# mdolab/dafoam

Hardware: NVIDIA H100
Metric: dRdWTPsi_GCells_per_s (higher is better)
Workload: dtype f64

## Files before the change

dafoam_b200/csrc/acc.hpp:

```cpp
#pragma once
#include "views.hpp"

namespace dab
{

struct GAcc
{
    MeshView m;
    StateView s;
    RecordView r;
    AdjView a;
    PsiView x;
    double *yU, *yP, *yN, *yPhi;

    DAB_HD int maxCF() const { return m.maxCF; }
    DAB_HD int nIF() const { return m.nIF; }
    DAB_HD FaceRef face(int c, int k) const { return faceOf(m, c, k); }
    template <int NF>
    DAB_HD void faceRow(int c, int* e, int* n) const
    {
        _Pragma("unroll") for (int k = 0; k < NF; k++)
        {
            e[k] = m.cellFaces[(size_t)k * m.nC + c];
            n[k] = m.cellNbr[(size_t)k * m.nC + c];
        }
    }
    DAB_HD bool ghost(int n) const { return n >= m.nC; }
    DAB_HD int patch(int f) const { return m.bPatch[f - m.nIF]; }
    DAB_HD void Sf(int f, double* v) const { v[0] = m.Sx[f]; v[1] = m.Sy[f]; v[2] = m.Sz[f]; }
    DAB_HD void kv(int f, double* v) const { v[0] = m.kx[f]; v[1] = m.ky[f]; v[2] = m.kz[f]; }
    DAB_HD void Cf(int f, double* v) const { v[0] = m.Cfx[f]; v[1] = m.Cfy[f]; v[2] = m.Cfz[f]; }
    DAB_HD double magSf(int f) const { return m.magSf[f]; }
    DAB_HD double w(int f) const { return m.w[f]; }
    DAB_HD double delta(int f) const { return m.delta[f]; }
    DAB_HD double phi(int f) const { return s.phi[f]; }
    DAB_HD double xphi(int f) const { return x.phi[f]; }
    DAB_HD double V(int c) const { return m.V[c]; }
    DAB_HD double yWall(int c) const { return m.yWall[c]; }
    DAB_HD double C(int c, int j) const { return (j == 0 ? m.Cx : (j == 1 ? m.Cy : m.Cz))[c]; }
    DAB_HD double U(int c, int j) const { return s.U[3 * c + j]; }
    DAB_HD double p(int c) const { return s.p[c]; }
    DAB_HD double nt(int c) const { return s.nt[c]; }
    DAB_HD double xU(int c, int j) const { return x.U[3 * c + j]; }
    DAB_HD double xp(int c) const { return x.p[c]; }
    DAB_HD double xnt(int c) const { return x.nt[c]; }
    DAB_HD double nut(int c) const { return r.nut[c]; }
    DAB_HD double gU(int c, int i) const { return r.gU[(size_t)i * m.nCtot + c]; }
    DAB_HD double gP(int c, int i) const { return r.gP[(size_t)i * m.nCtot + c]; }
    DAB_HD double gNt(int c, int i) const { return r.gNt[(size_t)i * m.nCtot + c]; }
    DAB_HD double rAU(int c) const { return r.rAU[c]; }
    DAB_HD double HbyA(int c, int j) const { return r.HbyA[(size_t)j * m.nCtot + c]; }
    DAB_HD double D0(int c) const { return r.D0[c]; }
    DAB_HD double flag(int c) const { return r.flag[c]; }
    DAB_HD double mt(int c, int j) const { return a.mt[(size_t)j * m.nCtot + c]; }
    DAB_HD double Dn(int c) const { return a.Dn[c]; }
    DAB_HD double Udir(int c, int j) const { return a.Udir[(size_t)j * m.nC + c]; }
    DAB_HD double pdir(int c) const { return a.pdir[c]; }
    DAB_HD double gPb(int c, int i) const { return a.gPb[(size_t)i * m.nCtot + c]; }
    DAB_HD double gUb(int c, int i) const { return a.gUb[(size_t)i * m.nCtot + c]; }
    DAB_HD double gNtb(int c, int i) const { return a.gNtb[(size_t)i * m.nCtot + c]; }
    DAB_HD double nutb(int c) const { return a.nutb[c]; }
    DAB_HD double U2(int c, int j) const { return a.U2[(size_t)j * m.nC + c]; }
    DAB_HD double nt2(int c) const { return a.nt2[c]; }
    DAB_HD void setMt(int c, int j, double v) const { a.mt[(size_t)j * m.nCtot + c] = v; }
    DAB_HD void setDn(int c, double v) const { a.Dn[c] = v; }
    DAB_HD void setUdir(int c, int j, double v) const { a.Udir[(size_t)j * m.nC + c] = v; }
    DAB_HD void setPdir(int c, double v) const { a.pdir[c] = v; }
    DAB_HD void setGPb(int c, int i, double v) const { a.gPb[(size_t)i * m.nCtot + c] = v; }
    DAB_HD void setGUb(int c, int i, double v) const { a.gUb[(size_t)i * m.nCtot + c] = v; }
    DAB_HD void setGNtb(int c, int i, double v) const { a.gNtb[(size_t)i * m.nCtot + c] = v; }
    DAB_HD void setNutb(int c, double v) const { a.nutb[c] = v; }
    DAB_HD void setU2(int c, int j, double v) const { a.U2[(size_t)j * m.nC + c] = v; }
// ... 14 lines not shown
```

dafoam_b200/csrc/rev_kernels.hpp:

```cpp
#pragma once
#include "views.hpp"
#include "acc.hpp"
#include "fwd_kernels.hpp"
#include <cmath>

namespace dab
{

DAB_HD double sgn(double x) { return x < 0.0 ? -1.0 : 1.0; }

DAB_HD void saSourceAdj(double nt, double nu, double y, const double* gU, const double* gN, double z, double& ntb, double* gUb, double* gNb, int fv3,
                        double* nub = nullptr)
{
    const double inu = frcp(nu);
    const double chi = nt * inu;
    const double c3 = chi * chi * chi, den1 = c3 + SA::Cv1c, iden1 = frcp(den1);
    const double fv1 = c3 * iden1;
    const double den = 1.0 + chi * fv1, iden = frcp(den);
    const double fv2 = 1.0 - chi * iden;
    const double w01 = 0.5 * (gU[3] - gU[1]), w02 = 0.5 * (gU[6] - gU[2]), w12 = 0.5 * (gU[7] - gU[5]);
    const double Q = w01 * w01 + w02 * w02 + w12 * w12;
    const double sQ = sqrt(Q);
    const double Omega = 2.0 * sQ;
    const double ky2 = (SA::kappa * y) * (SA::kappa * y), iky2 = frcp(ky2), iy2 = iky2 * (SA::kappa * SA::kappa);
// ... 228 lines not shown
    D0 = D1 + mt[0] * U[0] + mt[1] * U[1] + mt[2] * U[2];
}

template <int NF, int FEAT, class Acc>
DAB_HD void revBCell(const Acc& A, const Params& q, int c, bool gradOnly)
{
    const int schU = q.divU, schN = q.divNut;
    const double Uc[3] = {A.U(c, 0), A.U(c, 1), A.U(c, 2)};
    const double nuEc = A.nut(c) + q.nu;
    double gUc[9];
    for (int i = 0; i < 9; i++) gUc[i] = A.gU(c, i);
    const double ntc = q.turb ? A.nt(c) : 0.0;
    const double rsig = 1.0 / SA::sigma, rAl = frcp(q.alphaU);
    const double mtc[3] = {A.mt(c, 0), A.mt(c, 1), A.mt(c, 2)};
    const double Dnc = A.Dn(c), flc = A.flag(c);
    const double qc = (q.turb ? A.xnt(c) : 0.0) * (q.nrNut ? frcp(A.V(c)) : 1.0);

    double U2[3] = {0, 0, 0}, nt2 = 0.0, nuEb = 0.0, gUb[9], gNb[3] = {0, 0, 0};
    double refb[3] = {0, 0, 0};
    for (int i = 0; i < 9; i++) gUb[i] = 0.0;

    DAB_ACC_FACES(NF)
    int kb = NF > 0 ? NF : A.maxCF();
    _Pragma("unroll") for (int k = 0; k < (NF > 0 ? NF : A.maxCF()); k++)
    {
        const FaceRef fr = DAB_ACC_FACE(NF, k);
        if (fr.f < 0 || fr.bnd)
        {
            kb = k;
            break;
        }
        const int f = fr.f, n = fr.n;
        const double phi = A.phi(f), xphif = A.xphi(f);
        double Sv[3], kv[3], Cfv[3];
        A.Sf(f, Sv);
        A.kv(f, kv);
        A.Cf(f, Cfv);
        const double mS = A.magSf(f), dl = A.delta(f), wf = A.w(f);
        const double Un[3] = {A.U(n, 0), A.U(n, 1), A.U(n, 2)};
        const double nutn = A.nut(n), Dnn = A.Dn(n), fln = A.flag(n), Vn = A.V(n);
        const double mtn[3] = {A.mt(n, 0), A.mt(n, 1), A.mt(n, 2)};
        const double Cn[3] = {A.C(n, 0), A.C(n, 1), A.C(n, 2)};
        double gUn[9], gNn[3];
        for (int i = 0; i < 9; i++) gUn[i] = A.gU(n, i);
        const double ntn = q.turb ? A.nt(n) : 0.0, xntn = q.turb ? A.xnt(n) : 0.0;
        for (int i = 0; i < 3; i++) gNn[i] = q.turb ? A.gNt(n, i) : 0.0;
        const double Cc[3] = {A.C(c, 0), A.C(c, 1), A.C(c, 2)};
        double gNc[3];
        for (int i = 0; i < 3; i++) gNc[i] = q.turb ? A.gNt(c, i) : 0.0;
        const double mf = fr.s * phi;
        const double rmS = frcp(mS);
        double phib_acc = 0.0;
        const double wc = fr.s > 0 ? wf : 1.0 - wf, wn = 1.0 - wc;
        const bool pos0 = phi >= 0.0;
        const double wupc = fr.s > 0 ? (pos0 ? 1.0 : 0.0) : (pos0 ? 0.0 : 1.0);
        const double nuEn = nutn + q.nu;
        double D1c, soc, D0c, D1n, son, D0n;
        diagAdj(Dnc, flc, rAl, mtc, Uc, D1c, soc, D0c);
        diagAdj(Dnn, fln, rAl, mtn, Un, D1n, son, D0n);
        const bool ownUp = phi > 0.0;
        const bool cUp = fr.s > 0 ? ownUp : !ownUp;
        const double dC[3] = {Cfv[0] - Cc[0], Cfv[1] - Cc[1], Cfv[2] - Cc[2]};
        {
            const double wpc = schU == DIV_LINEAR ? wc : wupc;
            const double wpn = schU == DIV_LINEAR ? wn : 1.0 - wupc;
            const double gf = (wc * nuEc + wn * nuEn) * mS;
            const double g = gf * dl;
            const double offc = mf - wpc * mf - g;
            const double offn = -mf + wpn * mf - g;
            const double offbc = mtc[0] * Un[0] + mtc[1] * Un[1] + mtc[2] * Un[2] + sgn(offc) * soc;
            const double offbn = mtn[0] * Uc[0] + mtn[1] * Uc[1] + mtn[2] * Uc[2] + sgn(offn) * son;
            for (int j = 0; j < 3; j++) U2[j] += offn * mtn[j];
            const double abc = D0c - offbc, abn = D0n - offbn;
            double gb = abc + abn;
            double gfb = 0.0;
            const double lam[3] = {fr.s * (mtc[0] - mtn[0]), fr.s * (mtc[1] - mtn[1]), fr.s * (mtc[2] - mtn[2])};
            if (fr.s > 0)
            {
                const double mbc = -D0c + offbc + wpc * abc;
                const double mbn = -D0n + offbn + wpn * abn;
                phib_acc += mbc - mbn;
            }
            if (!(FEAT & 1))
            {
                if (schU == DIV_LINEAR_UPWIND)
                {
                    if (cUp)
                        for (int j = 0; j < 3; j++)
                            for (int i = 0; i < 3; i++) gUb[j * 3 + i] += dC[i] * phi * lam[j];
                    if (fr.s > 0)
                    {
                        double d[3];
                        for (int i = 0; i < 3; i++) d[i] = cUp ? dC[i] : Cfv[i] - Cn[i];
                        for (int j = 0; j < 3; j++)
                        {
                            const double gu0 = cUp ? gUc[j * 3 + 0] : gUn[j * 3 + 0], gu1 = cUp ? gUc[j * 3 + 1] : gUn[j * 3 + 1],
                                         gu2 = cUp ? gUc[j * 3 + 2] : gUn[j * 3 + 2];
                            phib_acc += (d[0] * gu0 + d[1] * gu1 + d[2] * gu2) * lam[j];
                        }
                    }
                }
            }
            else if (schU == DIV_LINEAR_UPWIND || schU == DIV_LINEAR_UPWIND_V)
            {
                double gu[9];
                for (int i = 0; i < 9; i++) gu[i] = cUp ? gUc[i] : gUn[i];
                double d[3];
                for (int i = 0; i < 3; i++) d[i] = cUp ? dC[i] : Cfv[i] - Cn[i];
                double corr[3], corrL[3], outb[3], corrb[3] = {0, 0, 0};
                for (int j = 0; j < 3; j++)
                {
                    corr[j] = d[0] * gu[j * 3 + 0] + d[1] * gu[j * 3 + 1] + d[2] * gu[j * 3 + 2];
                    outb[j] = phi * lam[j];
                }
                if ((FEAT & 1) && schU == DIV_LINEAR_UPWIND_V)
                {
                    const double cf = ownUp ? (1.0 - wf) : -wf;
                    double maxCorr[3], maxCorrb[3] = {0, 0, 0};
                    for (int j = 0; j < 3; j++) maxCorr[j] = cf * fr.s * (Un[j] - Uc[j]);
                    luvLimit(corr, maxCorr, corrL);
                    luvLimitAdj(corr, maxCorr, outb, corrb, maxCorrb);
                    for (int j = 0; j < 3; j++) U2[j] -= cf * fr.s * maxCorrb[j];
                }
                else
                    for (int j = 0; j < 3; j++) { corrL[j] = corr[j]; corrb[j] = outb[j]; }
                if (cUp)
                    for (int j = 0; j < 3; j++)
                        for (int i = 0; i < 3; i++) gUb[j * 3 + i] += dC[i] * corrb[j];
                if (fr.s > 0)
                    for (int j = 0; j < 3; j++) phib_acc += corrL[j] * lam[j];
            }
            for (int j = 0; j < 3; j++)
            {
                double cg = 0.0;
                for (int i = 0; i < 3; i++) cg += kv[i] * (wc * gUc[j * 3 + i] + wn * gUn[j * 3 + i]);
                gfb -= cg * lam[j];
                const double cgb = -gf * lam[j];
                for (int i = 0; i < 3; i++) gUb[j * 3 + i] += wc * kv[i] * cgb;
            }
            const double trc = gUc[0] + gUc[4] + gUc[8];
            double trb = 0.0;
            for (int j = 0; j < 3; j++)
            {
                const double tcb = -wc * lam[j];
                const double tcj = Sv[0] * gUc[0 * 3 + j] + Sv[1] * gUc[1 * 3 + j] + Sv[2] * gUc[2 * 3 + j] - (2.0 / 3.0) * trc * Sv[j];
                nuEb += tcb * tcj;
                for (int i = 0; i < 3; i++) gUb[i * 3 + j] += nuEc * Sv[i] * tcb;
                trb -= (2.0 / 3.0) * nuEc * Sv[j] * tcb;
            }
            gUb[0] += trb; gUb[4] += trb; gUb[8] += trb;
            nuEb += wc * mS * (dl * gb + gfb);
        }
        if (q.turb)
        {
            const double qn = xntn * (q.nrNut ? frcp(Vn) : 1.0);
            const double wpc = schN == DIV_LINEAR ? wc : wupc;
            const double wpn = schN == DIV_LINEAR ? wn : 1.0 - wupc;
            const double Gc = (ntc + q.nu) * rsig;
            const double gf = (wc * Gc + wn * (ntn + q.nu) * rsig) * mS;
            const double g = gf * dl;
            nt2 += qc * (wpc * mf + g - mf) + qn * (-mf + wpn * mf - g);
            const double gb = (qc - qn) * (ntc - ntn);
            double gfb = 0.0;
            const double lam = fr.s * (qc - qn);
            if (fr.s > 0) phib_acc += qc * (1.0 - wpc) * (ntn - ntc) - qn * (1.0 - wpn) * (ntc - ntn);
            if (schN == DIV_LINEAR_UPWIND)
            {
                if (cUp)
                    for (int i = 0; i < 3; i++) gNb[i] += dC[i] * phi * lam;
                if (fr.s > 0)
                {
                    double corr = 0.0;
                    for (int i = 0; i < 3; i++) corr += (cUp ? dC[i] * gNc[i] : (Cfv[i] - Cn[i]) * gNn[i]);
                    phib_acc += corr * lam;
                }
            }
            double cg = 0.0;
            for (int i = 0; i < 3; i++) cg += kv[i] * (wc * gNc[i] + wn * gNn[i]);
            gfb -= cg * lam;
            const double cgb = -gf * lam;
            for (int i = 0; i < 3; i++) gNb[i] += wc * kv[i] * cgb;
            nt2 += wc * mS * (dl * gb + gfb) * rsig;
        }
        if (!gradOnly)
        {
            if (fr.s > 0)
                A.setYPhi(f, (phib_acc - (q.nrPhi ? rmS : 1.0) * xphif) * phiRowScale(q, mS));
            else if (A.ghost(n))
                A.setYPhi(f, 0.0);
        }
    }
    _Pragma("unroll") for (int k = 0; k < (NF > 0 ? NF : A.maxCF()); k++)
    {
        if (k < kb) continue;
        const FaceRef fr = DAB_ACC_FACE(NF, k);
        if (fr.f < 0) break;
        const int f = fr.f;
        const double phi = A.phi(f), xphif = A.xphi(f);
        double Sv[3];
        A.Sf(f, Sv);
        const double mS = A.magSf(f), dl = A.delta(f);
        const int pa = A.patch(f);
        const double nutc = A.nut(c);
        const double mf = phi;
        const double rmS = frcp(mS);
        double D1c, soc, D0c;
// ... 390 lines not shown
```

dafoam_b200/csrc/solver.hpp:

```cpp
#pragma once
#include "backend.hpp"
#include "mesh.hpp"
#include "views.hpp"
#include "fwd_kernels.hpp"
#include "rev_kernels.hpp"
#include "tile_kernels.hpp"
#include "comp_kernels.hpp"
#include "comp_rev_kernels.hpp"
#include "krylov.hpp"
#include "primal_kernels.hpp"
#include "geom_kernels.hpp"
#include "comp_primal_kernels.hpp"
#include "launch_traits.hpp"
#include "partition.hpp"
#include "comm.hpp"
#include <chrono>
#include <cstdlib>
#include <cstdio>
#include <fstream>
#include <map>
#include <sys/stat.h>
#include <set>

namespace dab
// ... 135 lines not shown
    int pcExtraColourRadius = 0;
    int globalPCIters = 0;
    double richardsonOmega = 1.0;
    double gmresRelTol = 1e-6, gmresAbsTol = 1e-14, gmresTolDiff = 1e2, fdStep = 1e-6;
    std::string pcType = "ilu";
    std::string pcStorage = "fp64";
    int coarseAggregates = 0;
    int pcConLevel = 2;
    std::vector<FunctionDef> functions;
    std::vector<PatchVelocityDef> patchVelocities;
    std::vector<PatchVarDef> patchVars;
    FvSourceSpec fvSpec{};
    std::vector<std::string> diskNames;
    struct FvSourceParDef { std::string name, disk; std::vector<int> indices; };
    std::vector<FvSourceParDef> fvSourcePars;
    DevBuf<double> dFvS;
    struct MrfZone
    {
        bool on = false;
        std::string zone;
        double omega[3] = {0, 0, 0}, origin[3] = {0, 0, 0};
        std::vector<unsigned char> cell, type, faceIn;
    } mrf;
    DevBuf<unsigned char> dMrfCell, dMrfType, dMrfFaceIn;
    DevBuf<double> dMrfFlux;
    void updateMrfFlux()
    {
        if (mrf.on) be.launch(hm.nF, MrfFluxK{mv, dMrfFaceIn.p, dMrfFlux.p});
    }

    DevBuf<int32_t> dOwn, dNei, dCellFaces, dCellNbr, dBPatch;
    DevBuf<double> dS[3], dMagSf, dW, dDelta, dK[3], dCf[3], dV, dY;
    DevBuf<double> dC;
    MeshView mv;
    DevBuf<double> dWext, dU, dP, dNt, dPhi, dT;
    DevBuf<double> rRho, rNuL, rMuE, rAE, rHe, rEk, rGHe;
    DevBuf<double> aGHeb, aTdir, aCRho, aCNu, aCMuE, aCAE, aCHe, aCEk;
    StateView sv;
    DevBuf<double> rNut, rGU, rGP, rGNt, rRAU, rHbyA, rD0, rFlag;
    RecordView rv;
    DevBuf<double> aMt, aDn, aUdir, aPdir, aGPb, aGUb, aGNtb, aNutb, aU2, aNt2;
    AdjView av;
    DevBuf<double> dR, dX, dY2;
    bool recorded = false;
    Krylov kry;
    Comm comm;
    Halo halo;
    Partition part;
    DevBuf<double> psiP, psiN, psiPhi, psiT;

    TileMap tiles;
    DevBuf<int32_t> dTileCum, dTileGid, dTileTf, dTileTn;
    TileView tvw{};
    bool tilesOn = false;
    int tileCellsHint = 0;

    DevBuf<int32_t> dPfRanges;
    int pfChunks = 0;
    bool pfOn = false;

    bool fvSourceDirty = false;
    bool hex6 = false;
    int nCellStates() const { return 4 + (par.comp ? 1 : 0) + (par.turb ? 1 : 0); }
    int nDof() const { return nCellStates() * hm.nC + hm.nF; }
    void requireIncompressible(const char* what) const
    {
// ... 713 lines not shown
        (void)first;
        recorded = false;
    }

    void upload()
    {
        dOwn.upload(be, hm.own);
        dNei.upload(be, hm.nei);
        dCellFaces.upload(be, hm.cellFaces);
        hex6 = hm.maxCF == 6 && !(getenv("DAB_NOHEX6") && atoi(getenv("DAB_NOHEX6")) > 0);
        for (size_t i = 0; i < hm.cellFaces.size() && hex6; i++)
            if (hm.cellFaces[i] < 0) hex6 = false;
        hm.buildCellNbr();
        dCellNbr.upload(be, hm.cellNbr);
        dBPatch.upload(be, hm.bPatch);
        for (int k = 0; k < 3; k++)
        {
            dS[k].upload(be, hm.Sf[k]);
            dK[k].upload(be, hm.corr[k]);
            dCf[k].upload(be, hm.Cf[k]);
        }
        dC.alloc(be, (size_t)3 * hm.nCtot, false);
        for (int k = 0; k < 3; k++) be.h2d(dC.p + (size_t)k * hm.nCtot, hm.C[k].data(), (size_t)hm.nCtot * sizeof(double));
        dMagSf.upload(be, hm.magSf);
        dW.upload(be, hm.w);
        dDelta.upload(be, hm.delta);
        dV.upload(be, hm.V);
        dY.upload(be, hm.yWall);
        mv.nC = hm.nC; mv.nCtot = hm.nCtot; mv.nF = hm.nF; mv.nIF = hm.nIF; mv.nBF = hm.nBF; mv.maxCF = hm.maxCF;
        mv.own = dOwn.p; mv.nei = dNei.p; mv.cellFaces = dCellFaces.p; mv.cellNbr = dCellNbr.p; mv.bPatch = dBPatch.p;
        mv.Sx = dS[0].p; mv.Sy = dS[1].p; mv.Sz = dS[2].p; mv.magSf = dMagSf.p; mv.w = dW.p; mv.delta = dDelta.p;
        mv.kx = dK[0].p; mv.ky = dK[1].p; mv.kz = dK[2].p; mv.Cfx = dCf[0].p; mv.Cfy = dCf[1].p; mv.Cfz = dCf[2].p;
        mv.Cx = dC.p; mv.Cy = dC.p + hm.nCtot; mv.Cz = dC.p + 2 * (size_t)hm.nCtot; mv.V = dV.p; mv.yWall = dY.p;
        mv.fvS = nullptr;
        mv.mrfCell = nullptr; mv.mrfType = nullptr; mv.mrfFlux = nullptr;
        if (mrf.on)
        {
            dMrfCell.upload(be, mrf.cell);
            dMrfType.upload(be, mrf.type);
            dMrfFaceIn.upload(be, mrf.faceIn);
            dMrfFlux.alloc(be, hm.nF);
            for (int k = 0; k < 3; k++)
            {
                mv.mrfOmega[k] = mrf.omega[k];
                mv.mrfOrigin[k] = mrf.origin[k];
            }
            mv.mrfCell = dMrfCell.p; mv.mrfType = dMrfType.p; mv.mrfFlux = dMrfFlux.p;
            updateMrfFlux();
        }
        fvSourceDirty = fvSpec.nDisk > 0;
        const size_t nT = hm.nCtot, nC = hm.nC, nF = hm.nF, nd = nDof();
        dWext.alloc(be, nd);
        dU.alloc(be, 3 * nT); dP.alloc(be, nT); dNt.alloc(be, nT); dPhi.alloc(be, nF);
        sv.U = dU.p; sv.p = dP.p; sv.nt = dNt.p; sv.phi = dPhi.p; sv.T = nullptr;
        rv.rho = rv.nuL = rv.muE = rv.aE = rv.he = rv.Ek = rv.gHe = nullptr;
        if (par.comp)
        {
            dT.alloc(be, nT);
            sv.T = dT.p;
            rRho.alloc(be, nT); rNuL.alloc(be, nT); rMuE.alloc(be, nT); rAE.alloc(be, nT); rHe.alloc(be, nT); rEk.alloc(be, nT);
            rGHe.alloc(be, 3 * nT);
            rv.rho = rRho.p; rv.nuL = rNuL.p; rv.muE = rMuE.p; rv.aE = rAE.p; rv.he = rHe.p; rv.Ek = rEk.p; rv.gHe = rGHe.p;
        }
        rNut.alloc(be, nT); rGU.alloc(be, 9 * nT); rGP.alloc(be, 3 * nT); rGNt.alloc(be, 3 * nT);
        rRAU.alloc(be, nT); rHbyA.alloc(be, 3 * nT); rD0.alloc(be, nT); rFlag.alloc(be, nT);
        rv.nut = rNut.p; rv.gU = rGU.p; rv.gP = rGP.p; rv.gNt = rGNt.p; rv.rAU = rRAU.p; rv.HbyA = rHbyA.p; rv.D0 = rD0.p; rv.flag = rFlag.p;
// ... 107 lines not shown
        PfPlan pl;
        if (!pfOn) return pl;
        pl.nC = hm.nC;
        pl.nChunks = pfChunks;
        pl.ranges = dPfRanges.p;
        static const int ahead = getenv("DAB_PF_AHEAD") ? atoi(getenv("DAB_PF_AHEAD")) : 0;
        pl.ahead = ahead;
        const size_t nC = hm.nC;
        for (int k = 0; k < hm.maxCF && k < 6; k++)
        {
            pl.cell(mv.cellFaces + (size_t)k * nC, 4);
            pl.cell(mv.cellNbr + (size_t)k * nC, 4);
        }
        return pl;
    }
    PfPlan pfRevA(const PsiView& pv) const
    {
        PfPlan pl = pfBase();
        if (!pfOn) return pl;
        const size_t nT = hm.nCtot;
        pl.cell(sv.U, 24); pl.cell(pv.U, 24); pl.cell(pv.p, 8); pl.cell(mv.V, 8); pl.cell(sv.p, 8); pl.cell(rv.rAU, 8); pl.cell(rv.D0, 8);
        for (int j = 0; j < 3; j++) { pl.cell(rv.gP + j * nT, 8); pl.cell(rv.HbyA + j * nT, 8); }
        pl.face(mv.magSf, 8); pl.face(mv.delta, 8); pl.face(mv.Sx, 8); pl.face(mv.Sy, 8); pl.face(mv.Sz, 8); pl.face(pv.phi, 8);
        pl.face(mv.w, 8); pl.face(mv.kx, 8); pl.face(mv.ky, 8); pl.face(mv.kz, 8); pl.face(sv.phi, 8);
        return pl;
    }
    PfPlan pfRevB(const PsiView& pv) const
    {
        PfPlan pl = pfBase();
        if (!pfOn) return pl;
        const size_t nT = hm.nCtot;
        pl.cell(sv.U, 24); pl.cell(rv.nut, 8); pl.cell(mv.V, 8); pl.cell(av.Dn, 8); pl.cell(rv.flag, 8);
        for (int i = 0; i < 9; i++) pl.cell(rv.gU + i * nT, 8);
        for (int j = 0; j < 3; j++) { pl.cell(av.mt + j * nT, 8); pl.cell((j == 0 ? mv.Cx : (j == 1 ? mv.Cy : mv.Cz)), 8); }
        if (par.turb)
        {
            pl.cell(sv.nt, 8); pl.cell(pv.nt, 8); pl.cell(mv.yWall, 8);
            for (int j = 0; j < 3; j++) pl.cell(rv.gNt + j * nT, 8);
        }
        pl.face(sv.phi, 8); pl.face(mv.Sx, 8); pl.face(mv.Sy, 8); pl.face(mv.Sz, 8); pl.face(mv.magSf, 8); pl.face(mv.delta, 8); pl.face(mv.w, 8);
        pl.face(mv.kx, 8); pl.face(mv.ky, 8); pl.face(mv.kz, 8); pl.face(mv.Cfx, 8); pl.face(mv.Cfy, 8); pl.face(mv.Cfz, 8); pl.face(pv.phi, 8);
        return pl;
    }
    PfPlan pfRevC() const
    {
        PfPlan pl = pfBase();
        if (!pfOn) return pl;
        const size_t nT = hm.nCtot, nC = hm.nC;
        pl.cell(av.pdir, 8); pl.cell(mv.V, 8);
        for (int j = 0; j < 3; j++) { pl.cell(av.Udir + j * nC, 8); pl.cell(av.U2 + j * nC, 8); pl.cell(av.gPb + j * nT, 8); }
        for (int i = 0; i < 9; i++) pl.cell(av.gUb + i * nT, 8);
        if (par.turb)
        {
            pl.cell(av.nt2, 8); pl.cell(av.nutb, 8); pl.cell(sv.nt, 8);
            for (int j = 0; j < 3; j++) pl.cell(av.gNtb + j * nT, 8);
        }
        pl.face(mv.Sx, 8); pl.face(mv.Sy, 8); pl.face(mv.Sz, 8); pl.face(mv.w, 8); pl.face(sv.phi, 8); pl.face(mv.delta, 8); pl.face(mv.magSf, 8);
        return pl;
    }

    void calcPCMatWithFvMatrix(int turbOnly, std::vector<int32_t>& rows, std::vector<int32_t>& cols, std::vector<double>& vals)
    {
        if (!turbOnly)
            throw Error("calcPCMatWithFvMatrix: only turbOnly = 1 is available for " + solverName
                        + " (the reference's DAResidual::calcPCMatWithFvMatrix aborts for the SIMPLE solver family)");
        rows.clear(); cols.clear(); vals.clear();
        if (!par.turb) return;
        if (par.comp) throw Error("calcPCMatWithFvMatrix: the compressible nuTilda matrix export is not built (DASimpleFoam only)");
        ensureRecorded();
        const int nC = hm.nC, nIF = hm.nIF, mcf = hm.maxCF;
        DevBuf<double> off, diag, b;
        off.alloc(be, (size_t)mcf * nC);
        diag.alloc(be, nC);
        b.alloc(be, nC);
// ... 1050 lines not shown
            fprintf(f, "    }\n");
        }
        fprintf(f, "}\n");
        fclose(f);
        return std::sqrt(norm2);
    }

    void writeMeshPoints(const double* pts, const std::string& dirName) const
    {
        if (ghosted()) throw Error("mesh output needs an undecomposed mesh without cyclic patches in this build");
        const std::string d1 = caseDirectory + "/" + dirName, d2 = d1 + "/polyMesh";
        ::mkdir(d1.c_str(), 0755);
        ::mkdir(d2.c_str(), 0755);
        FILE* f = fopen((d2 + "/points").c_str(), "w");
        if (!f) throw Error("cannot write " + d2 + "/points");
        fprintf(f, "FoamFile\n{\n    version 2.0;\n    format ascii;\n    class vectorField;\n    location \"%s/polyMesh\";\n    object points;\n}\n\n%d\n(\n",
                dirName.c_str(), hm.nP);
        for (int i = 0; i < hm.nP; i++) fprintf(f, "(%.17g %.17g %.17g)\n", pts[3 * i], pts[3 * i + 1], pts[3 * i + 2]);
        fprintf(f, ")\n");
        fclose(f);
    }
    void readMeshPoints(const std::string& timeName)
    {
        std::vector<double> pts;
        readVectorField(caseDirectory + "/" + timeName + "/polyMesh/points", pts);
        if (pts.size() != hm.points.size()) throw Error("readMeshPoints: " + timeName + "/polyMesh/points has the wrong size");
        updateMesh(pts.data());
    }
    void readStateVars(const std::string& timeName) { initialStates(caseDirectory, timeName); }

    VolCoord volc;
    void uploadGeometry();
    void deviceGeometry();
    void downloadGeometry();
    void updateMesh(const double* pts);
    void volCoordSetup();
    void volCoordProduct(const double* psi, const FunctionDef* function, double seed, double* out);

    Primal primal;
    VecOps primalOps;
    void primalSetup();
    const double* primalSums(int k);
    void primalResidual(const EqnView& e, const double* x, const double* g, double* res);
    void primalJacobi(const EqnView& e, double* x, double* tmp, const double* g, const SegControl& ctl, double* res0);
    void primalCoarseSetup();
    void primalCoarseRefresh(const EqnView& e);
    void primalPrecond(const EqnView& e, const double* r, double* z);
    int primalPcg(const EqnView& e, double* x, const SegControl& ctl, double& res0);
    int solvePrimal(PrimalStats& st);

    void pcSymbolic();
    void calcPC();
    void applyPC(const double* v, double* z);
    void applyIlu(const double* v, double* z);
    void coarseSetup();
    void coarseRestrict(const double* v, bool toHost = true);
    int kspExtraMatvecs = 0;
    int solveLinearEqn(const double* rhs, double* sol, KspStats& st);
    int solveIdrs(const double* rhs, double* sol, KspStats& st);
    int solveFixedPoint(const double* rhs, double* sol, KspStats& st);
};

}

#include "solver_krylov.hpp"
#include "solver_primal.hpp"
// ... 2 lines not shown
```

dafoam_b200/csrc/solver_volcoord.hpp:

```cpp
#pragma once

namespace dab
{

inline void Solver::uploadGeometry()
{
    auto put = [&](double* d, const std::vector<double>& h) { be.h2d(d, h.data(), h.size() * sizeof(double)); };
    for (int k = 0; k < 3; k++)
    {
        put(dS[k].p, hm.Sf[k]);
        put(dK[k].p, hm.corr[k]);
        put(dCf[k].p, hm.Cf[k]);
        put(dC.p + (size_t)k * hm.nCtot, hm.C[k]);
    }
    put(dMagSf.p, hm.magSf);
    put(dW.p, hm.w);
    put(dDelta.p, hm.delta);
    put(dV.p, hm.V);
    updateMrfFlux();
    recorded = false;
    kry.pcValid = false;
}

inline void Solver::downloadGeometry()
{
    auto get = [&](std::vector<double>& h, const double* d) { be.d2h(h.data(), d, h.size() * sizeof(double)); };
    for (int k = 0; k < 3; k++)
    {
        get(hm.Sf[k], dS[k].p);
        get(hm.corr[k], dK[k].p);
        get(hm.Cf[k], dCf[k].p);
        get(hm.C[k], dC.p + (size_t)k * hm.nCtot);
    }
    get(hm.magSf, dMagSf.p);
    get(hm.w, dW.p);
    get(hm.delta, dDelta.p);
    get(hm.V, dV.p);
}

inline void Solver::deviceGeometry()
{
    VolCoord& Vc = volc;
    if (!Vc.topoReady)
    {
        Vc.dFOff.upload(be, hm.fOff);
        Vc.dFLab.upload(be, hm.fLab);
        if (hm.hasCyclic()) Vc.dFaceXf.upload(be, part.faceXf);
        Vc.topoReady = true;
    }
    const size_t nT = hm.nCtot;
    GeomView gv;
    gv.nC = hm.nC; gv.nF = hm.nF; gv.nIF = hm.nIF; gv.maxCF = hm.maxCF;
    gv.fOff = Vc.dFOff.p; gv.fLab = Vc.dFLab.p; gv.own = dOwn.p; gv.nei = dNei.p; gv.cellFaces = dCellFaces.p;
    gv.pts = Vc.dPts.p;
    gv.Sx = dS[0].p; gv.Sy = dS[1].p; gv.Sz = dS[2].p; gv.magSf = dMagSf.p; gv.w = dW.p; gv.delta = dDelta.p;
    gv.kx = dK[0].p; gv.ky = dK[1].p; gv.kz = dK[2].p; gv.Cfx = dCf[0].p; gv.Cfy = dCf[1].p; gv.Cfz = dCf[2].p;
    gv.Cx = dC.p; gv.Cy = dC.p + nT; gv.Cz = dC.p + 2 * nT; gv.V = dV.p;
    gv.faceXf = Vc.dFaceXf.n ? Vc.dFaceXf.p : nullptr;
    gv.Rtab = halo.dRtab.p;
    gv.Ttab = halo.dTtab.p;
    be.launch(hm.nF, GeomFaceK{gv});
    be.launch(hm.nC, GeomCellK{gv});
    if (ghosted())
    {
        HaloItem centres{dC.p, 3, 1, (int)nT};
        centres.position = true;
        halo.exchangeCells({centres, {dV.p, 1, 1, (int)nT}});
    }
    be.launch(hm.nF, GeomDerivedK{gv});
}

inline void Solver::updateMesh(const double* pts)
{
    const std::vector<double> old(hm.points);
    std::copy(pts, pts + hm.points.size(), hm.points.begin());
    if (!ghosted())
        hm.computeGeometry();
    else
    {
        try
        {
            hm.checkCyclicPairs();
        }
        catch (...)
        {
            hm.points = old;
            throw;
        }
        if (volc.dPts.n != hm.points.size()) volc.dPts.alloc(be, hm.points.size(), false);
        be.h2d(volc.dPts.p, hm.points.data(), hm.points.size() * sizeof(double));
        deviceGeometry();
        downloadGeometry();
    }
    uploadGeometry();
    fvSourceDirty = fvSpec.nDisk > 0;
    if (volc.ready) be.h2d(volc.dPts0.p, hm.points.data(), hm.points.size() * sizeof(double));
}

inline void Solver::volCoordSetup()
{
    VolCoord& Vc = volc;
    if (Vc.ready) return;
// ... 218 lines not shown
```

dafoam_b200/csrc/tile_kernels.hpp:

```cpp
#pragma once
#include "rev_kernels.hpp"
#include "tiles.hpp"

namespace dab
{

constexpr int TILE_TMAX = 192;
constexpr int TILE_EXT1 = 256;
constexpr int TILE_EXT2 = 320;

struct TAccBase
{
    MeshView m;
    StateView s;
    PsiView x;
    double* sm;
    const int32_t *tf, *tn;
    int ln, c0, maxCF_;
    DAB_HD int maxCF() const { return maxCF_; }
    DAB_HD int nIF() const { return m.nIF; }
    DAB_HD FaceRef face(int c, int k) const { return faceOfE2(m.nIF, tf[(size_t)k * ln + c], tn[(size_t)k * ln + c]); }
    template <int NF>
    DAB_HD void faceRow(int c, int* e, int* n) const
    {
        _Pragma("unroll") for (int k = 0; k < NF; k++)
        {
            e[k] = tf[(size_t)k * ln + c];
            n[k] = tn[(size_t)k * ln + c];
        }
    }
    DAB_HD bool ghost(int) const { return false; }
    DAB_HD int patch(int f) const { return m.bPatch[f - m.nIF]; }
    DAB_HD void Sf(int f, double* v) const { v[0] = m.Sx[f]; v[1] = m.Sy[f]; v[2] = m.Sz[f]; }
    DAB_HD void kv(int f, double* v) const { v[0] = m.kx[f]; v[1] = m.ky[f]; v[2] = m.kz[f]; }
    DAB_HD void Cf(int f, double* v) const { v[0] = m.Cfx[f]; v[1] = m.Cfy[f]; v[2] = m.Cfz[f]; }
    DAB_HD double magSf(int f) const { return m.magSf[f]; }
    DAB_HD double w(int f) const { return m.w[f]; }
    DAB_HD double delta(int f) const { return m.delta[f]; }
    DAB_HD double phi(int f) const { return s.phi[f]; }
    DAB_HD double xphi(int f) const { return x.phi[f]; }
    DAB_HD bool mrfCell(int) const { return false; }
    DAB_HD bool bcRefOn(int) const { return false; }
    DAB_HD bool bcRefAny() const { return false; }
    DAB_HD void setBcRef(int, int, double) const {}
    DAB_HD void addBcRef(int, int, double) const {}
};

struct TAccA : TAccBase
{
    static constexpr int E1 = TILE_EXT1;
    enum { O_XP = 0, O_V = E1, O_GP = 2 * E1, O_P = 5 * E1, O_RAU = 6 * E1, SM_DOUBLES = 7 * E1 };
    RecordView r;
    AdjView a;
    int nTg, nCg;
    DAB_HD double V(int c) const { return sm[O_V + c]; }
    DAB_HD double xp(int c) const { return sm[O_XP + c]; }
    DAB_HD double gP(int c, int i) const { return sm[O_GP + i * E1 + c]; }
    DAB_HD double p(int c) const { return sm[O_P + c]; }
    DAB_HD double rAU(int c) const { return sm[O_RAU + c]; }
    DAB_HD double U(int c, int j) const { return s.U[3 * (size_t)(c0 + c) + j]; }
    DAB_HD double xU(int c, int j) const { return x.U[3 * (size_t)(c0 + c) + j]; }
    DAB_HD double HbyA(int c, int j) const { return r.HbyA[(size_t)j * nTg + c0 + c]; }
    DAB_HD double D0(int c) const { return r.D0[c0 + c]; }
    DAB_HD void setMt(int c, int j, double v) const { a.mt[(size_t)j * nTg + c0 + c] = v; }
    DAB_HD void setDn(int c, double v) const { a.Dn[c0 + c] = v; }
    DAB_HD void setUdir(int c, int j, double v) const { a.Udir[(size_t)j * nCg + c0 + c] = v; }
    DAB_HD void setPdir(int c, double v) const { a.pdir[c0 + c] = v; }
    DAB_HD void setGPb(int c, int i, double v) const { a.gPb[(size_t)i * nTg + c0 + c] = v; }
// ... 20 lines not shown
        const int n0 = cum[0], n1 = cum[1];
        const int c0 = t * tv.T;
        const int nTg = m.nCtot;
        if (ph == 0)
        {
            const int32_t* gid = tv.gid + (size_t)t * tv.ls;
            for (int l = tid; l < n1; l += nthr)
            {
                const int g = l < n0 ? c0 + l : gid[l];
                sm[TAccA::O_XP + l] = x.p[g];
                sm[TAccA::O_V + l] = m.V[g];
                for (int i = 0; i < 3; i++) sm[TAccA::O_GP + i * E1 + l] = r.gP[(size_t)i * nTg + g];
                sm[TAccA::O_P + l] = s.p[g];
                sm[TAccA::O_RAU + l] = r.rAU[g];
            }
            return;
        }
        TAccA A;
        A.m = m; A.s = s; A.x = x; A.sm = sm;
        A.tf = tv.tf + (size_t)t * tv.maxCF * tv.ln;
        A.tn = tv.tn + (size_t)t * tv.maxCF * tv.ln;
        A.ln = tv.ln; A.c0 = c0; A.maxCF_ = tv.maxCF;
        A.r = r; A.a = a; A.nTg = nTg; A.nCg = m.nC;
        for (int l = tid; l < n0; l += nthr) revACell<NF>(A, q, l);
    }
};

struct TAccBC : TAccBase
{
    static constexpr int E1 = TILE_EXT1, E2 = TILE_EXT2, TM = TILE_TMAX;
    enum
    {
        O_U = 0, O_NUT = 3 * E2, O_MT = 4 * E2, O_DN = 7 * E2, O_FLAG = 8 * E2, O_GU = 9 * E2, O_NT = 18 * E2, O_XNT = 19 * E2,
        O_V = 20 * E2, O_GNT = 21 * E2, O_C = 24 * E2, END2 = 27 * E2,
        O_GPB = END2, O_GUB = END2 + 3 * E1, O_GNTB = END2 + 12 * E1, O_YW = END2 + 15 * E1, END1 = END2 + 16 * E1,
        O_U2 = END1, O_NT2 = END1 + 3 * TM, O_NUTB = END1 + 4 * TM, SM_DOUBLES = END1 + 5 * TM
    };
    AdjView a;
    double *yU, *yP, *yN, *yPhi;
    int nCg;
    DAB_HD double U(int c, int j) const { return sm[O_U + j * E2 + c]; }
    DAB_HD double nut(int c) const { return sm[O_NUT + c]; }
    DAB_HD double mt(int c, int j) const { return sm[O_MT + j * E2 + c]; }
    DAB_HD double Dn(int c) const { return sm[O_DN + c]; }
    DAB_HD double flag(int c) const { return sm[O_FLAG + c]; }
    DAB_HD double gU(int c, int i) const { return sm[O_GU + i * E2 + c]; }
    DAB_HD double nt(int c) const { return sm[O_NT + c]; }
    DAB_HD double xnt(int c) const { return sm[O_XNT + c]; }
    DAB_HD double V(int c) const { return sm[O_V + c]; }
    DAB_HD double gNt(int c, int i) const { return sm[O_GNT + i * E2 + c]; }
    DAB_HD double C(int c, int j) const { return sm[O_C + j * E2 + c]; }
    DAB_HD double yWall(int c) const { return sm[O_YW + c]; }
    DAB_HD double gPb(int c, int i) const { return sm[O_GPB + i * E1 + c]; }
    DAB_HD double gUb(int c, int i) const { return sm[O_GUB + i * E1 + c]; }
    DAB_HD double gNtb(int c, int i) const { return sm[O_GNTB + i * E1 + c]; }
    DAB_HD double U2(int c, int j) const { return sm[O_U2 + j * TM + c]; }
    DAB_HD double nt2(int c) const { return sm[O_NT2 + c]; }
    DAB_HD double nutb(int c) const { return sm[O_NUTB + c]; }
    DAB_HD void setGUb(int c, int i, double v) const { sm[O_GUB + i * E1 + c] = v; }
    DAB_HD void setGNtb(int c, int i, double v) const { sm[O_GNTB + i * E1 + c] = v; }
    DAB_HD void setU2(int c, int j, double v) const { sm[O_U2 + j * TM + c] = v; }
    DAB_HD void setNt2(int c, double v) const { sm[O_NT2 + c] = v; }
    DAB_HD void setNutb(int c, double v) const { sm[O_NUTB + c] = v; }
    DAB_HD double Udir(int c, int j) const { return a.Udir[(size_t)j * nCg + c0 + c]; }
    DAB_HD double pdir(int c) const { return a.pdir[c0 + c]; }
    DAB_HD void setYU(int c, int j, double v) const { yU[3 * (size_t)(c0 + c) + j] = v; }
    DAB_HD void setYP(int c, double v) const { yP[c0 + c] = v; }
    DAB_HD void setYN(int c, double v) const { yN[c0 + c] = v; }
    DAB_HD void setYPhi(int f, double v) const { yPhi[f] = v; }
};

template <int NF, int FEAT>
struct ProdTileBC
{
    static constexpr int THREADS = TILE_TMAX;
    static constexpr int MAXREG = 168;
    static constexpr int PHASES = 3;
    static constexpr int SM_DOUBLES = TAccBC::SM_DOUBLES;
    MeshView m;
    Params q;
    StateView s;
    RecordView r;
    AdjView a;
    PsiView x;
    double* y;
    TileView tv;
    DAB_HD void phase(int ph, int t, int tid, int nthr, double* sm) const
    {
        constexpr int E1 = TILE_EXT1, E2 = TILE_EXT2;
        const int32_t* cum = tv.cum + (size_t)t * (tv.R + 1);
        const int n0 = cum[0], n1 = cum[1], n2 = cum[2];
        const int c0 = t * tv.T;
        const int nTg = m.nCtot;
        if (ph == 0)
        {
            const int32_t* gid = tv.gid + (size_t)t * tv.ls;
            for (int l = tid; l < n2; l += nthr)
            {
                const int g = l < n0 ? c0 + l : gid[l];
                for (int j = 0; j < 3; j++) sm[TAccBC::O_U + j * E2 + l] = s.U[3 * (size_t)g + j];
                sm[TAccBC::O_NUT + l] = r.nut[g];
                for (int j = 0; j < 3; j++) sm[TAccBC::O_MT + j * E2 + l] = a.mt[(size_t)j * nTg + g];
                sm[TAccBC::O_DN + l] = a.Dn[g];
                sm[TAccBC::O_FLAG + l] = r.flag[g];
                for (int i = 0; i < 9; i++) sm[TAccBC::O_GU + i * E2 + l] = r.gU[(size_t)i * nTg + g];
                sm[TAccBC::O_NT + l] = q.turb ? s.nt[g] : 0.0;
                sm[TAccBC::O_XNT + l] = q.turb ? x.nt[g] : 0.0;
                sm[TAccBC::O_V + l] = m.V[g];
                for (int i = 0; i < 3; i++) sm[TAccBC::O_GNT + i * E2 + l] = q.turb ? r.gNt[(size_t)i * nTg + g] : 0.0;
                sm[TAccBC::O_C + l] = m.Cx[g];
                sm[TAccBC::O_C + E2 + l] = m.Cy[g];
                sm[TAccBC::O_C + 2 * E2 + l] = m.Cz[g];
                if (l < n1)
                {
                    for (int i = 0; i < 3; i++) sm[TAccBC::O_GPB + i * E1 + l] = a.gPb[(size_t)i * nTg + g];
                    sm[TAccBC::O_YW + l] = m.yWall[g];
                }
            }
            return;
        }
        TAccBC A;
        A.m = m; A.s = s; A.x = x; A.sm = sm;
        A.tf = tv.tf + (size_t)t * tv.maxCF * tv.ln;
        A.tn = tv.tn + (size_t)t * tv.maxCF * tv.ln;
        A.ln = tv.ln; A.c0 = c0; A.maxCF_ = tv.maxCF;
        A.a = a; A.nCg = m.nC;
        const size_t nC = m.nC;
        A.yU = y; A.yP = y + 3 * nC; A.yN = y + 4 * nC; A.yPhi = y + (size_t)(q.turb ? 5 : 4) * nC;
        if (ph == 1)
        {
            for (int l = tid; l < n1; l += nthr) revBCell<NF, FEAT>(A, q, l, l >= n0);
            return;
        }
        for (int l = tid; l < n0; l += nthr) revCCell<NF>(A, q, l, 0);
    }
};

}
```

dafoam_b200/csrc/views.hpp:

```cpp
#pragma once
#include <cmath>
#include <cstdint>

#if defined(__CUDACC__)
#define DAB_HD __host__ __device__ __forceinline__
#else
#define DAB_HD inline
#endif

namespace dab
{

DAB_HD double frcp(double x)
{
#if defined(__CUDA_ARCH__)
    double r;
    asm("rcp.approx.ftz.f64 %0, %1;" : "=d"(r) : "d"(x));
    r = fma(fma(-x, r, 1.0), r, r);
    r = fma(fma(-x, r, 1.0), r, r);
    return r;
#else
    return 1.0 / x;
#endif
}

constexpr int MAXP = 16;
enum { F_U = 0, F_P = 1, F_NUTILDA = 2, F_NUT = 3, N_FIELDS = 4 };
enum { BC_FIXED_VALUE = 0, BC_ZERO_GRADIENT = 1, BC_INLET_OUTLET = 2, BC_OUTLET_INLET = 3, BC_SYMMETRY = 4, BC_CALCULATED = 5, BC_NUT_LOW_RE = 6, BC_NUT_SPALDING = 7 };
enum { DIV_UPWIND = 0, DIV_LINEAR_UPWIND = 1, DIV_LINEAR = 2, DIV_LINEAR_UPWIND_V = 3, DIV_LIMITED_LINEAR = 4  };

struct MeshView
{
    int nC, nCtot, nF, nIF, nBF, maxCF;
    const int32_t* own;
    const int32_t* nei;
    const int32_t* cellFaces;
    const int32_t* cellNbr;
    const int32_t* bPatch;
    const double *Sx, *Sy, *Sz, *magSf, *w, *delta, *kx, *ky, *kz, *Cfx, *Cfy, *Cfz;
    const double *Cx, *Cy, *Cz, *V, *yWall;
    const double* fvS;
    const unsigned char* mrfCell;
    const unsigned char* mrfType;
    const double* mrfFlux;
    double mrfOmega[3], mrfOrigin[3];
};

DAB_HD void mrfWallRef(const MeshView& m, int f, const double* patchVal, double* ref)
{
    ref[0] = patchVal[0];
    ref[1] = patchVal[1];
    ref[2] = patchVal[2];
    if (m.mrfType && m.mrfType[f - m.nIF] == 1)
    {
        const double r[3] = {m.Cfx[f] - m.mrfOrigin[0], m.Cfy[f] - m.mrfOrigin[1], m.Cfz[f] - m.mrfOrigin[2]};
        const double* w = m.mrfOmega;
        ref[0] = w[1] * r[2] - w[2] * r[1];
        ref[1] = w[2] * r[0] - w[0] * r[2];
        ref[2] = w[0] * r[1] - w[1] * r[0];
    }
}

DAB_HD double mrfBoundaryFlux(const MeshView& m, int f, double ph, double rhob)
{
    if (!m.mrfType) return ph;
    const int ty = m.mrfType[f - m.nIF];
    return ty == 1 ? 0.0 : (ty == 2 ? ph - rhob * m.mrfFlux[f] : ph);
}

struct MrfFluxK
{
    MeshView m;
    const unsigned char* faceIn;
    double* out;
    DAB_HD void operator()(int f) const
    {
        double v = 0.0;
        if (faceIn[f])
        {
            const double r[3] = {m.Cfx[f] - m.mrfOrigin[0], m.Cfy[f] - m.mrfOrigin[1], m.Cfz[f] - m.mrfOrigin[2]};
            const double* w = m.mrfOmega;
            v = (w[1] * r[2] - w[2] * r[1]) * m.Sx[f] + (w[2] * r[0] - w[0] * r[2]) * m.Sy[f] + (w[0] * r[1] - w[1] * r[0]) * m.Sz[f];
        }
        out[f] = v;
    }
};

struct ActuatorDisk
{
    double par[13];
    double eps;
    int rotLeft;
};
constexpr int MAXDISK = 4;
struct FvSourceSpec
{
    int nDisk;
    ActuatorDisk disk[MAXDISK];
};

DAB_HD void actuatorDiskSource(const ActuatorDisk& d, const double* C, double* out)
{
    const double* a = d.par;
    const double dm = sqrt(a[3] * a[3] + a[4] * a[4] + a[5] * a[5]);
    const double dn[3] = {a[3] / dm, a[4] / dm, a[5] / dm};
    const double rin = a[6], rout = a[7], scale = a[8], POD = a[9], expM = a[10], expN = a[11], eps = d.eps;
    const double epsR = eps / (rout - rin), rMin = epsR, rMax = 1.0 - epsR;
    const double fRMin = pow(rMin, expM) * pow(1.0 - rMin, expN), fRMax = pow(rMax, expM) * pow(1.0 - rMax, expN);
    const double v[3] = {C[0] - a[0], C[1] - a[1], C[2] - a[2]};
    const double vA[3] = {v[0] * dn[0], v[1] * dn[1], v[2] * dn[2]};
    const double vR[3] = {v[0] - vA[0], v[1] - vA[1], v[2] - vA[2]};
    double vC[3];
    if (d.rotLeft) { vC[0] = vR[1] * dn[2] - vR[2] * dn[1]; vC[1] = vR[2] * dn[0] - vR[0] * dn[2]; vC[2] = vR[0] * dn[1] - vR[1] * dn[0]; }
    else { vC[0] = dn[1] * vR[2] - dn[2] * vR[1]; vC[1] = dn[2] * vR[0] - dn[0] * vR[2]; vC[2] = dn[0] * vR[1] - dn[1] * vR[0]; }
    const double rLen = sqrt(vR[0] * vR[0] + vR[1] * vR[1] + vR[2] * vR[2]);
    const double cLen = sqrt(vC[0] * vC[0] + vC[1] * vC[1] + vC[2] * vC[2]);
    const double dA2 = vA[0] * vA[0] + vA[1] * vA[1] + vA[2] * vA[2];
    const double rPrime = rLen / rout, rHub = rin / rout;
    const double rStar = (rPrime - rHub) / (1.0 - rHub);
// ... 397 lines not shown
```

Baseline: 1.245.

## Precompute per-face owner/neighbour centre offsets for reverse adjoint kernel

Adds a per-internal-face buffer holding face-centre minus owner and neighbour cell-centre vectors, refreshed whenever geometry changes. The reverse kernel reads these offsets instead of gathering cell centres for both cells plus face centres, and the tiled variant drops cell centres from shared memory. This cuts irregular cell-centre gathers and shared-memory footprint, at the cost of six face-sized reads per face instead of three face reads plus gathers, and an extra buffer to keep in sync with mesh updates.

```diff
diff --git a/dafoam_b200/csrc/acc.hpp b/dafoam_b200/csrc/acc.hpp
--- a/dafoam_b200/csrc/acc.hpp
+++ b/dafoam_b200/csrc/acc.hpp
@@ -29,7 +29,7 @@
     DAB_HD int patch(int f) const { return m.bPatch[f - m.nIF]; }
     DAB_HD void Sf(int f, double* v) const { v[0] = m.Sx[f]; v[1] = m.Sy[f]; v[2] = m.Sz[f]; }
     DAB_HD void kv(int f, double* v) const { v[0] = m.kx[f]; v[1] = m.ky[f]; v[2] = m.kz[f]; }
-    DAB_HD void Cf(int f, double* v) const { v[0] = m.Cfx[f]; v[1] = m.Cfy[f]; v[2] = m.Cfz[f]; }
+    DAB_HD void faceOff(int f, double* dO, double* dN) const { faceOffsets(m, f, dO, dN); }
     DAB_HD double magSf(int f) const { return m.magSf[f]; }
     DAB_HD double w(int f) const { return m.w[f]; }
     DAB_HD double delta(int f) const { return m.delta[f]; }
@@ -37,7 +37,6 @@
     DAB_HD double xphi(int f) const { return x.phi[f]; }
     DAB_HD double V(int c) const { return m.V[c]; }
     DAB_HD double yWall(int c) const { return m.yWall[c]; }
-    DAB_HD double C(int c, int j) const { return (j == 0 ? m.Cx : (j == 1 ? m.Cy : m.Cz))[c]; }
     DAB_HD double U(int c, int j) const { return s.U[3 * c + j]; }
     DAB_HD double p(int c) const { return s.p[c]; }
     DAB_HD double nt(int c) const { return s.nt[c]; }
diff --git a/dafoam_b200/csrc/rev_kernels.hpp b/dafoam_b200/csrc/rev_kernels.hpp
--- a/dafoam_b200/csrc/rev_kernels.hpp
+++ b/dafoam_b200/csrc/rev_kernels.hpp
@@ -284,20 +284,18 @@
         }
         const int f = fr.f, n = fr.n;
         const double phi = A.phi(f), xphif = A.xphi(f);
-        double Sv[3], kv[3], Cfv[3];
+        double Sv[3], kv[3], dO[3], dN[3];
         A.Sf(f, Sv);
         A.kv(f, kv);
-        A.Cf(f, Cfv);
+        A.faceOff(f, dO, dN);
         const double mS = A.magSf(f), dl = A.delta(f), wf = A.w(f);
         const double Un[3] = {A.U(n, 0), A.U(n, 1), A.U(n, 2)};
         const double nutn = A.nut(n), Dnn = A.Dn(n), fln = A.flag(n), Vn = A.V(n);
         const double mtn[3] = {A.mt(n, 0), A.mt(n, 1), A.mt(n, 2)};
-        const double Cn[3] = {A.C(n, 0), A.C(n, 1), A.C(n, 2)};
         double gUn[9], gNn[3];
         for (int i = 0; i < 9; i++) gUn[i] = A.gU(n, i);
         const double ntn = q.turb ? A.nt(n) : 0.0, xntn = q.turb ? A.xnt(n) : 0.0;
         for (int i = 0; i < 3; i++) gNn[i] = q.turb ? A.gNt(n, i) : 0.0;
-        const double Cc[3] = {A.C(c, 0), A.C(c, 1), A.C(c, 2)};
         double gNc[3];
         for (int i = 0; i < 3; i++) gNc[i] = q.turb ? A.gNt(c, i) : 0.0;
         const double mf = fr.s * phi;
@@ -312,7 +310,8 @@
         diagAdj(Dnn, fln, rAl, mtn, Un, D1n, son, D0n);
         const bool ownUp = phi > 0.0;
         const bool cUp = fr.s > 0 ? ownUp : !ownUp;
-        const double dC[3] = {Cfv[0] - Cc[0], Cfv[1] - Cc[1], Cfv[2] - Cc[2]};
+        const double dC[3] = {fr.s > 0 ? dO[0] : dN[0], fr.s > 0 ? dO[1] : dN[1], fr.s > 0 ? dO[2] : dN[2]};
+        const double dX[3] = {fr.s > 0 ? dN[0] : dO[0], fr.s > 0 ? dN[1] : dO[1], fr.s > 0 ? dN[2] : dO[2]};
         {
             const double wpc = schU == DIV_LINEAR ? wc : wupc;
             const double wpn = schU == DIV_LINEAR ? wn : 1.0 - wupc;
@@ -343,7 +342,7 @@
                     if (fr.s > 0)
                     {
                         double d[3];
-                        for (int i = 0; i < 3; i++) d[i] = cUp ? dC[i] : Cfv[i] - Cn[i];
+                        for (int i = 0; i < 3; i++) d[i] = cUp ? dC[i] : dX[i];
                         for (int j = 0; j < 3; j++)
                         {
                             const double gu0 = cUp ? gUc[j * 3 + 0] : gUn[j * 3 + 0], gu1 = cUp ? gUc[j * 3 + 1] : gUn[j * 3 + 1],
@@ -358,7 +357,7 @@
                 double gu[9];
                 for (int i = 0; i < 9; i++) gu[i] = cUp ? gUc[i] : gUn[i];
                 double d[3];
-                for (int i = 0; i < 3; i++) d[i] = cUp ? dC[i] : Cfv[i] - Cn[i];
+                for (int i = 0; i < 3; i++) d[i] = cUp ? dC[i] : dX[i];
                 double corr[3], corrL[3], outb[3], corrb[3] = {0, 0, 0};
                 for (int j = 0; j < 3; j++)
                 {
@@ -423,7 +422,7 @@
                 if (fr.s > 0)
                 {
                     double corr = 0.0;
-                    for (int i = 0; i < 3; i++) corr += (cUp ? dC[i] * gNc[i] : (Cfv[i] - Cn[i]) * gNn[i]);
+                    for (int i = 0; i < 3; i++) corr += (cUp ? dC[i] * gNc[i] : dX[i] * gNn[i]);
                     phib_acc += corr * lam;
                 }
             }
diff --git a/dafoam_b200/csrc/solver.hpp b/dafoam_b200/csrc/solver.hpp
--- a/dafoam_b200/csrc/solver.hpp
+++ b/dafoam_b200/csrc/solver.hpp
@@ -191,6 +191,7 @@
     DevBuf<int32_t> dOwn, dNei, dCellFaces, dCellNbr, dBPatch;
     DevBuf<double> dS[3], dMagSf, dW, dDelta, dK[3], dCf[3], dV, dY;
     DevBuf<double> dC;
+    DevBuf<double> dFaceOff;
     MeshView mv;
     DevBuf<double> dWext, dU, dP, dNt, dPhi, dT;
     DevBuf<double> rRho, rNuL, rMuE, rAE, rHe, rEk, rGHe;
@@ -970,6 +971,9 @@
         mv.Sx = dS[0].p; mv.Sy = dS[1].p; mv.Sz = dS[2].p; mv.magSf = dMagSf.p; mv.w = dW.p; mv.delta = dDelta.p;
         mv.kx = dK[0].p; mv.ky = dK[1].p; mv.kz = dK[2].p; mv.Cfx = dCf[0].p; mv.Cfy = dCf[1].p; mv.Cfz = dCf[2].p;
         mv.Cx = dC.p; mv.Cy = dC.p + hm.nCtot; mv.Cz = dC.p + 2 * (size_t)hm.nCtot; mv.V = dV.p; mv.yWall = dY.p;
+        dFaceOff.alloc(be, (size_t)6 * hm.nIF, false);
+        mv.offOwn = dFaceOff.p; mv.offNei = dFaceOff.p + (size_t)3 * hm.nIF;
+        updateFaceOffsets();
         mv.fvS = nullptr;
         mv.mrfCell = nullptr; mv.mrfType = nullptr; mv.mrfFlux = nullptr;
         if (mrf.on)
@@ -1143,14 +1147,14 @@
         const size_t nT = hm.nCtot;
         pl.cell(sv.U, 24); pl.cell(rv.nut, 8); pl.cell(mv.V, 8); pl.cell(av.Dn, 8); pl.cell(rv.flag, 8);
         for (int i = 0; i < 9; i++) pl.cell(rv.gU + i * nT, 8);
-        for (int j = 0; j < 3; j++) { pl.cell(av.mt + j * nT, 8); pl.cell((j == 0 ? mv.Cx : (j == 1 ? mv.Cy : mv.Cz)), 8); }
+        for (int j = 0; j < 3; j++) pl.cell(av.mt + j * nT, 8);
         if (par.turb)
         {
             pl.cell(sv.nt, 8); pl.cell(pv.nt, 8); pl.cell(mv.yWall, 8);
             for (int j = 0; j < 3; j++) pl.cell(rv.gNt + j * nT, 8);
         }
         pl.face(sv.phi, 8); pl.face(mv.Sx, 8); pl.face(mv.Sy, 8); pl.face(mv.Sz, 8); pl.face(mv.magSf, 8); pl.face(mv.delta, 8); pl.face(mv.w, 8);
-        pl.face(mv.kx, 8); pl.face(mv.ky, 8); pl.face(mv.kz, 8); pl.face(mv.Cfx, 8); pl.face(mv.Cfy, 8); pl.face(mv.Cfz, 8); pl.face(pv.phi, 8);
+        pl.face(mv.kx, 8); pl.face(mv.ky, 8); pl.face(mv.kz, 8); pl.face(pv.phi, 8);
         return pl;
     }
     PfPlan pfRevC() const
@@ -2267,6 +2271,7 @@
     VolCoord volc;
     void uploadGeometry();
     void deviceGeometry();
+    void updateFaceOffsets() { be.launch(hm.nIF, FaceOffsetK{mv, dFaceOff.p, dFaceOff.p + (size_t)3 * hm.nIF}); }
     void downloadGeometry();
     void updateMesh(const double* pts);
     void volCoordSetup();
diff --git a/dafoam_b200/csrc/solver_volcoord.hpp b/dafoam_b200/csrc/solver_volcoord.hpp
--- a/dafoam_b200/csrc/solver_volcoord.hpp
+++ b/dafoam_b200/csrc/solver_volcoord.hpp
@@ -17,6 +17,7 @@
     put(dW.p, hm.w);
     put(dDelta.p, hm.delta);
     put(dV.p, hm.V);
+    updateFaceOffsets();
     updateMrfFlux();
     recorded = false;
     kry.pcValid = false;
@@ -68,6 +69,7 @@
         halo.exchangeCells({centres, {dV.p, 1, 1, (int)nT}});
     }
     be.launch(hm.nF, GeomDerivedK{gv});
+    updateFaceOffsets();
 }
 
 inline void Solver::updateMesh(const double* pts)
diff --git a/dafoam_b200/csrc/tile_kernels.hpp b/dafoam_b200/csrc/tile_kernels.hpp
--- a/dafoam_b200/csrc/tile_kernels.hpp
+++ b/dafoam_b200/csrc/tile_kernels.hpp
@@ -33,7 +33,7 @@
     DAB_HD int patch(int f) const { return m.bPatch[f - m.nIF]; }
     DAB_HD void Sf(int f, double* v) const { v[0] = m.Sx[f]; v[1] = m.Sy[f]; v[2] = m.Sz[f]; }
     DAB_HD void kv(int f, double* v) const { v[0] = m.kx[f]; v[1] = m.ky[f]; v[2] = m.kz[f]; }
-    DAB_HD void Cf(int f, double* v) const { v[0] = m.Cfx[f]; v[1] = m.Cfy[f]; v[2] = m.Cfz[f]; }
+    DAB_HD void faceOff(int f, double* dO, double* dN) const { faceOffsets(m, f, dO, dN); }
     DAB_HD double magSf(int f) const { return m.magSf[f]; }
     DAB_HD double w(int f) const { return m.w[f]; }
     DAB_HD double delta(int f) const { return m.delta[f]; }
@@ -120,7 +120,7 @@
     enum
     {
         O_U = 0, O_NUT = 3 * E2, O_MT = 4 * E2, O_DN = 7 * E2, O_FLAG = 8 * E2, O_GU = 9 * E2, O_NT = 18 * E2, O_XNT = 19 * E2,
-        O_V = 20 * E2, O_GNT = 21 * E2, O_C = 24 * E2, END2 = 27 * E2,
+        O_V = 20 * E2, O_GNT = 21 * E2, END2 = 24 * E2,
         O_GPB = END2, O_GUB = END2 + 3 * E1, O_GNTB = END2 + 12 * E1, O_YW = END2 + 15 * E1, END1 = END2 + 16 * E1,
         O_U2 = END1, O_NT2 = END1 + 3 * TM, O_NUTB = END1 + 4 * TM, SM_DOUBLES = END1 + 5 * TM
     };
@@ -137,7 +137,6 @@
     DAB_HD double xnt(int c) const { return sm[O_XNT + c]; }
     DAB_HD double V(int c) const { return sm[O_V + c]; }
     DAB_HD double gNt(int c, int i) const { return sm[O_GNT + i * E2 + c]; }
-    DAB_HD double C(int c, int j) const { return sm[O_C + j * E2 + c]; }
     DAB_HD double yWall(int c) const { return sm[O_YW + c]; }
     DAB_HD double gPb(int c, int i) const { return sm[O_GPB + i * E1 + c]; }
     DAB_HD double gUb(int c, int i) const { return sm[O_GUB + i * E1 + c]; }
@@ -196,9 +195,6 @@
                 sm[TAccBC::O_XNT + l] = q.turb ? x.nt[g] : 0.0;
                 sm[TAccBC::O_V + l] = m.V[g];
                 for (int i = 0; i < 3; i++) sm[TAccBC::O_GNT + i * E2 + l] = q.turb ? r.gNt[(size_t)i * nTg + g] : 0.0;
-                sm[TAccBC::O_C + l] = m.Cx[g];
-                sm[TAccBC::O_C + E2 + l] = m.Cy[g];
-                sm[TAccBC::O_C + 2 * E2 + l] = m.Cz[g];
                 if (l < n1)
                 {
                     for (int i = 0; i < 3; i++) sm[TAccBC::O_GPB + i * E1 + l] = a.gPb[(size_t)i * nTg + g];
diff --git a/dafoam_b200/csrc/views.hpp b/dafoam_b200/csrc/views.hpp
--- a/dafoam_b200/csrc/views.hpp
+++ b/dafoam_b200/csrc/views.hpp
@@ -39,6 +39,7 @@
     const int32_t* bPatch;
     const double *Sx, *Sy, *Sz, *magSf, *w, *delta, *kx, *ky, *kz, *Cfx, *Cfy, *Cfz;
     const double *Cx, *Cy, *Cz, *V, *yWall;
+    const double *offOwn, *offNei;
     const double* fvS;
     const unsigned char* mrfCell;
     const unsigned char* mrfType;
@@ -85,6 +86,32 @@
         out[f] = v;
     }
 };
+
+struct FaceOffsetK
+{
+    MeshView m;
+    double *offOwn, *offNei;
+    DAB_HD void operator()(int f) const
+    {
+        const size_t nIF = m.nIF;
+        const int o = m.own[f], n = m.nei[f];
+        offOwn[f] = m.Cfx[f] - m.Cx[o]; offOwn[nIF + f] = m.Cfy[f] - m.Cy[o]; offOwn[2 * nIF + f] = m.Cfz[f] - m.Cz[o];
+        offNei[f] = m.Cfx[f] - m.Cx[n]; offNei[nIF + f] = m.Cfy[f] - m.Cy[n]; offNei[2 * nIF + f] = m.Cfz[f] - m.Cz[n];
+    }
+};
+
+DAB_HD void faceOffsets(const MeshView& m, int f, double* dO, double* dN)
+{
+#if defined(DAB_FACE_OFFSETS_FROM_CENTRES)
+    const int o = m.own[f], n = m.nei[f];
+    dO[0] = m.Cfx[f] - m.Cx[o]; dO[1] = m.Cfy[f] - m.Cy[o]; dO[2] = m.Cfz[f] - m.Cz[o];
+    dN[0] = m.Cfx[f] - m.Cx[n]; dN[1] = m.Cfy[f] - m.Cy[n]; dN[2] = m.Cfz[f] - m.Cz[n];
+#else
+    const size_t nIF = m.nIF;
+    dO[0] = m.offOwn[f]; dO[1] = m.offOwn[nIF + f]; dO[2] = m.offOwn[2 * nIF + f];
+    dN[0] = m.offNei[f]; dN[1] = m.offNei[nIF + f]; dN[2] = m.offNei[2 * nIF + f];
+#endif
+}
 
 struct ActuatorDisk
 {
```

After: 1.285 (median of 6 runs). 1.03x the previous value.
